# autowarefoundation/autoware_vision_pilot

Hardware: AMD Instinct MI355X
Metric: frames/sec (SceneSeg+Scene3D 1280x720, one camera per GPU: preprocess + shared encoder + 2 decoder(s) + decode per frame); p50 per-frame latency beside it (higher is better)
Workload: dtype fp16x3 (hi+lo fp16 pairs on the fp16 MFMA pipe, fp32 accumulate; fp32-class: floats within 1e-3 of the fp32 oracle, 0 class flips outside that float tolerance -- tie flips only, counted per pass in profiles/r06_parity_sweep.tsv)

## Files before the change

### autoware_vision_pilot_amd/csrc/engine_upconv.cpp

```cpp
#include "engine_internal.hpp"

namespace vp {

namespace {

inline void tap_of(int q, int tt, int* a, int* d) {
  const int hr = q + tt - 1;
  const int o = hr >= 0 ? hr / 2 : -1;
  *d = hr - 2 * o;
  *a = o + 1 - q;
}

inline void split_half_d(double v, double pre, half_t* hi, half_t* lo) {
  const double x = v * pre;
  if (!(std::fabs(x) <= 65504.0)) throw RangeError("composed up-sampling weight " + std::to_string(v) + " is outside the fp16 range the matrix pipe carries: re-scale the checkpoint");
  const half_t h = (half_t)x;
  *hi = h;
  *lo = truncate_lo((half_t)(x - (double)h));
}

}

void Engine::compose_upconv(const float* wt, const float* bt, const float* ws, const float* bs, const float* w3, const float* b3, int cin, int cm, int cout,
                            int cs, UpconvComposed* out) {
// ... 141 lines not shown
      }
      for (int t = 0; t < 9 && cs > 0; ++t) {
        const double* row = cw.ws.data() + ((size_t)t * cout + co) * cs;
        for (int c = 0; c < cs; ++c) amax = std::max(amax, std::fabs(row[c]));
      }
      const int sexp = prescale_exp((float)amax);
      const double pre = std::ldexp(1.0, sexp);
      post[(size_t)phase * coutw + co] = std::ldexp(1.0f, -sexp);
      for (int c = 0; c < n_chunks; ++c) {
        const UpconvChunk d = upconv_chunk(c, py, px, cin_v, cs_v);
        const int creal = d.skip ? cs : cin;
        for (int k = 0; k < d.nt; ++k) {
          const int a = d.a0 + (d.nb == 2 ? (k >> 1) : k), b = d.b0 + (d.nb == 2 ? (k & 1) : 0);
          const double* row;
          if (d.skip) {
            const int ty = d.qy != py ? 2 * a : 1, tx = d.qx != px ? 2 * b : 1;
            row = cw.ws.data() + ((size_t)(ty * 3 + tx) * cout + co) * cs;
          } else {
            row = cw.wx.data() + ((size_t)(phase * 4 + a * 2 + b) * cout + co) * cin;
          }
          for (int i = 0; i < chunk_w && chm * d.ch0 + i < creal; ++i) {
            const size_t dst = upconv_pack_index(phase, d.step0 + k, co, i & 31, S, coutw);
            if (x1) {
              half_t h, l;
              split_half_d(row[chm * d.ch0 + i], pre, &h, &l);
              (i >> 5 ? lo : hi)[dst] = h;
            } else {
              split_half_d(row[d.ch0 + i], pre, &hi[dst], &lo[dst]);
            }
          }
        }
      }
    }
  });
  Act* out = new_act(out_name.empty() ? name : out_name, cout, in->H * 2, in->W * 2);
  UpconvParams p{};
  p.in_hi = in->hi;
  p.in_lo = x1 ? nullptr : in->lo;
  p.sk_hi = skip_in ? skip_in->hi : nullptr;
  p.sk_lo = (skip_in && !x1) ? skip_in->lo : nullptr;
  p.H = in->H;
  p.W = in->W;
  p.Cin = cin_pad;
  p.Cs = cs_pad;
  p.w_hi = dupload(hi);
  p.w_lo = dupload(lo);
  wbytes_[1] += 2 * (hi.size() + lo.size());
  p.bias = dupload(bias);
  p.wscale = dupload(post);
  p.CoutW = coutw;
  p.Ncols = ncols;
  p.Cstore = out->C;
  p.out_hi = out->hi;
  p.out_lo = x1 ? nullptr : out->lo;
  p.act = (x1 && act == ACT_GELU) ? ACT_GELU_F16 : act;
  const long long t16 = (long long)((in->H + 15) / 16) * ((in->W + 15) / 16), t8 = (long long)((in->H + 7) / 8) * ((in->W + 15) / 16);
  const int n_co = coutw / 128;
  int sh = shape;
  {
    int ot = -1, on = 0;
    if (sh < 0 && plan_override(name, &ot, &on)) {
      sh = ot;
      if (on > 0 && nsplit <= 0) nsplit = on;
    }
  }
  if (sh < 0) {
    const double eff6 = (double)in->H * in->W / (double)(t16 * 256), eff7 = (double)in->H * in->W / (double)(t8 * 128);
    const char* e = dev_option("VP_UPCONV_SHAPE");
    sh = e ? std::atoi(e) : ((eff7 > 1.1 * eff6 || cin_pad <= 128) ? 7 : 6);
  }
  if (sh != 6 && sh != 7) throw std::invalid_argument("composed up-sampling stage: shape 6 (16x16 patches, 8 waves) or 7 (8x16 patches, 4 waves): " + name);
  const long long blocks = (sh == 6 ? t16 : t8) * 4 * n_co;
  int ns = nsplit;
  if (ns <= 0) {
    const long long slots = sh == 6 ? 256 : 512;
    ns = (int)std::max<long long>(1, slots / blocks);
    const double slice_mb = 4.0 * in->H * in->W * coutw * 4.0 / 1e6;
    while (ns > 1 && ns * slice_mb > 26.0) --ns;
    while (ns > 1 && S / ns < 12) --ns;
    if (const char* e = dev_option("VP_UPCONV_NSPLIT")) ns = std::max(1, std::atoi(e));
  }
  ns = std::max(1, std::min(ns, n_chunks));
  p.nsplit = ns;
  p.partial = ns > 1 ? static_cast<float*>(dalloc((size_t)ns * 4 * in->H * in->W * coutw * sizeof(float), false)) : nullptr;
  if (!upconv_supported(p, sh)) throw std::invalid_argument("composed up-sampling stage: shape not covered: " + name);
  Op op;
  op.name = name;
  op.kernel = std::string(x1 ? "upconv_x1" : "upconv_x3") + (sh == 6 ? "w8<co128,px256" : "w4<co128,px128") + (x1 ? ",k64>" : ">") + (ns > 1 ? "+splitk" : "");
  if (ns > 1) op.launch = "nsplit=" + std::to_string(ns);
  const double M2 = 4.0 * in->H * in->W;
  op.flops = 2.0 * (M2 * cin * cm + M2 * cs * cm + M2 * 9.0 * cm * cout);
  op.flops_executed = 2.0 * M2 * cout * (4.0 * cin + 9.0 * cs);
  op.bytes = (x1 ? 2.0 : 4.0) * ((M2 / 4 * cin + M2 * cs + M2 * cout) + cout * (16.0 * cin + 9.0 * cs));
  op.run = [p, sh](hipStream_t st) { return launch_upconv(p, sh, st); };
  ops_.push_back(std::move(op));
  return out;
}

}
```

### autoware_vision_pilot_amd/csrc/kernels.hpp

```cpp
#pragma once
#include "common.hpp"

namespace vp {

const char* dev_option(const char* key);
bool dev_option_is(const char* key, char first);

struct PreprocessParams {
  const uint8_t* frame;
  int stride;
  const int* xtab;
  const int* ytab;
  int out_h, out_w;
  int src_c[3];
  float mean[3], stdv[3];
  float* out;
  int norm_form;
};

struct PilResampleParams {
  const uint8_t* frame;
  int stride;
  int in_h, in_w, out_h, out_w;
  const int* hb;
// ... 126 lines not shown
  int N, K, act;
  unsigned act_rows;
  int rows_kernel;
  const float* partial;
  int nslab, Kstride;
  float inv_hw;
};

bool fc_rows_ok(const FcParams& p);

struct CtxConv1Params {
  const float* map;
  int H, W;
  const float* w;
  const float* b;
  ActView out;
  int act;
};

struct CtxExpConv1Params {
  FcParams fc;
  CtxConv1Params cv;
  int tile;
  int glanes;
};
bool ctx_exp_conv1_ok(const CtxExpConv1Params& p);
hipError_t launch_ctx_exp_conv1(const CtxExpConv1Params& p, hipStream_t st);

struct FusionParams {
  ActView f[5];
  int creal[5];
  int shift[5];
  ActView out;
  int Creal_out;
  int octets;
};
bool fusion_octets_ok(const FusionParams& p);

hipError_t launch_conv_gemm(const ConvGemmParams& p, int tile, int bk, bool split, hipStream_t st);
int conv_tile_co(int tile);
int conv_tile_px(int tile);
hipError_t launch_conv3x3_halo(const ConvGemmParams& p, int tile, bool split, hipStream_t st);
bool conv3x3_x3_supported(const ConvGemmParams& p, int shape);
hipError_t launch_conv3x3_x3(const ConvGemmParams& p, int shape, hipStream_t st);
int halo_tile_co(int tile);
int halo_tile_px(int tile);
int halo_tile_th(int tile);

int conv3x3_map_geometry(int H, int W);
bool conv3x3_map_shape_ok(int H, int W, int cin_pad, int coutw);
size_t conv3x3_map_pack_index(int co, int ci, int t, int cin_pad);
size_t conv3x3_map_pack_index_k32(int co, int ci, int t, int cin_pad);
bool conv3x3_map_supported(const ConvGemmParams& p);
hipError_t launch_conv3x3_map(const ConvGemmParams& p, hipStream_t st);
bool conv3x3_map2_shape_ok(int H, int W, int cin_pad, int coutw);
bool conv3x3_map2_supported(const ConvGemmParams& p);
size_t conv3x3_map2_pack_index(int co, int ci, int t, int cin_pad);
hipError_t launch_conv3x3_map2(const ConvGemmParams& p, hipStream_t st);
bool head_conv_supported(const ConvGemmParams& p);
hipError_t launch_head_conv(const ConvGemmParams& p, const void* zeros, hipStream_t st);
bool gemm_dma_shape_ok(int M, int ncols, int cin_pad, int cin2_pad, int cstore);
size_t gemm_dma_pack_index(int n, int k, int kw);
bool gemm_dma_supported(const ConvGemmParams& p, bool split);
hipError_t launch_gemm_dma(const ConvGemmParams& p, hipStream_t st);
bool convt_rs_supported(const ConvGemmParams& p, bool split);
int convt_rs_shape_case(int H, int W, int cin_pad, int cin2_pad, int ncols, int cstore);
hipError_t launch_convt_rs(const ConvGemmParams& p, hipStream_t st);
struct UpconvParams {
  const half_t* in_hi;
  const half_t* in_lo;
  const half_t* sk_hi;
  const half_t* sk_lo;
  int H, W, Cin, Cs;
  const half_t* w_hi;
  const half_t* w_lo;
  const float* bias;
  const float* wscale;
  int CoutW, Ncols, Cstore;
  half_t* out_hi;
  half_t* out_lo;
  int act;
  int nsplit;
  float* partial;
};
bool upconv_supported(const UpconvParams& p, int shape);
struct UpconvChunk {
  int skip, ch0, qy, qx, nt, nb, a0, b0, step0;
};
__host__ __device__ inline UpconvChunk upconv_chunk(int c, int py, int px, int cin_pad, int cs_pad) {
  const int kcx = cin_pad >> 5, kcs = cs_pad >> 5;
  UpconvChunk d;
  if (c < kcx || kcs == 0) {
    d.skip = 0; d.ch0 = c << 5; d.qy = 0; d.qx = 0; d.nt = 4; d.nb = 2; d.a0 = 0; d.b0 = 0; d.step0 = 4 * c;
    return d;
  }
  const int r = c - kcx, cls = r / kcs, cc = r - cls * kcs;
  d.skip = 1;
  d.ch0 = cc << 5;
  d.qy = cls < 2 ? 1 - py : py;
  d.qx = (cls & 1) ? px : 1 - px;
  const int na = d.qy != py ? 2 : 1;
  d.nb = d.qx != px ? 2 : 1;
  d.a0 = na == 2 ? 0 : 1 - py;
  d.b0 = d.nb == 2 ? 0 : 1 - px;
  d.nt = na * d.nb;
  const int cls_step0 = cls == 0 ? 0 : (cls == 1 ? 4 : (cls == 2 ? 6 : 8));
  d.step0 = 4 * kcx + cls_step0 * kcs + cc * d.nt;
  return d;
}
__host__ __device__ inline int upconv_chunks(int cin_pad, int cs_pad) { return (cin_pad >> 5) + 4 * (cs_pad >> 5); }
__host__ __device__ inline int upconv_steps(int cin_pad, int cs_pad) { return 4 * (cin_pad >> 5) + 9 * (cs_pad >> 5); }
inline size_t upconv_pack_index(int phase, int step, int co, int i, int steps, int coutw) {
  const int i_sw = ((((i & 31) >> 3) ^ ((co >> 2) & 3)) << 3) | (i & 7);
  return (((size_t)phase * steps + step) * coutw + co) * 32 + i_sw;
}
hipError_t launch_upconv(const UpconvParams& p, int shape, hipStream_t st);
struct ComposeGemmParams {
  const float* a[4];
  const float* b[4];
  int pairs, M, N, K;
  double* c;
};
hipError_t launch_compose_gemm(const ComposeGemmParams* groups_dev, int n_groups, int M, int N, hipStream_t st);
hipError_t launch_preprocess(const PreprocessParams& p, hipStream_t st);
hipError_t launch_pil_resample(const PilResampleParams& p, hipStream_t st);
hipError_t launch_stem(const StemParams& p, hipStream_t st);
hipError_t launch_dwconv(const DwParams& p, hipStream_t st);
bool mbconv_front_supported(const MbFrontParams& p);
hipError_t launch_mbconv_front(const MbFrontParams& p, hipStream_t st);
hipError_t launch_letterbox(const LetterboxParams& p, hipStream_t st);
hipError_t launch_detect_decode_nms(const DetectParams& p, hipStream_t st);
bool mbconv_back_supported(const MbBackParams& p);
hipError_t launch_mbconv_back(const MbBackParams& p, hipStream_t st);
hipError_t launch_pool_partial(const PoolParams& p, hipStream_t st);
hipError_t launch_zero_u64(unsigned long long* p, size_t n, hipStream_t st);
constexpr int kSeMaxReplicas = 64;
hipError_t launch_se_gate_scale(const SeParams& se, const ScaleWParams& sw, hipStream_t st);
hipError_t launch_fc(const FcParams& p, hipStream_t st);
hipError_t launch_ctx_conv1(const CtxConv1Params& p, hipStream_t st);
hipError_t launch_fusion(const FusionParams& p, hipStream_t st);
hipError_t launch_decode_mask(const float* logits, int C, int HW, int mode, uint8_t* out, hipStream_t st);
hipError_t launch_resize_nearest(const uint8_t* src, int sw, const int* ytab, const int* xtab, int oh, int ow, uint8_t* dst,
                                 hipStream_t st);
hipError_t launch_resize_bilinear_f32(const float* src, int sw, const int* yi, const float* yf, const int* xi, const float* xf,
                                      int oh, int ow, float* dst, hipStream_t st);
hipError_t launch_minmax_f32(const float* src, size_t n, unsigned* mm, hipStream_t st);
constexpr int VP_PROBE_BLOCKS = 64;
hipError_t launch_finite_probe(const float* src, size_t n, unsigned* flags, hipStream_t st);
hipError_t launch_depth_colorize(const float* src, size_t n, const unsigned* mm, const uint8_t* lut, uint8_t* dst, hipStream_t st);
hipError_t launch_viz_blend(const uint8_t* mask, int mw, const int* ytab, const int* xtab, const uint8_t* frame, int stride, int oh, int ow,
                            const uint8_t* lut, int frame_is_rgb, uint8_t* dst, hipStream_t st);
hipError_t launch_nchw_to_act(const float* src, int Creal, const ActView& a, hipStream_t st);
hipError_t launch_act_to_nchw(const ActView& a, int Creal, float* dst, hipStream_t st);

hipError_t launch_chan_copy(const ActView& src, int src_off, const ActView& dst, int dst_off, int nch, hipStream_t st);
hipError_t launch_maxpool5(const ActView& src, int src_off, const ActView& dst, int dst_off, int nch, hipStream_t st);
bool sppf_pool_ok(const ActView& src, const ActView& dst, int nch);
hipError_t launch_sppf_pool(const ActView& src, const ActView& dst, int nch, hipStream_t st);
struct AttnParams {
  ActView qkv;
  ActView out;
  ActView vout;
  int heads, dk, dv;
  float scale;
  int qblock;
};
bool attention_block_ok(const AttnParams& p);
hipError_t launch_attention(const AttnParams& p, hipStream_t st);
// ... 10 lines not shown
```

### autoware_vision_pilot_amd/csrc/kernels_upconv.hip

```cpp
#include <algorithm>
#include <cstdlib>

#include "conv_epilogue.hpp"
#include "lds_dma.hpp"

namespace vp {

namespace {

struct PixPhase {
  int y0, x0, H, W, py, px;
  __device__ __forceinline__ int operator()(int q) const {
    int rowbit, c;
    lane_to_px16(q & 31, rowbit, c);
    const int y = y0 + 2 * (q >> 5) + rowbit, x = x0 + c;
    return (y < H && x < W) ? (2 * y + py) * (2 * W) + 2 * x + px : -1;
  }
};
__device__ __forceinline__ int bias_class(int m, int H2, int W2) {
  const int Y = m / W2, X = m - Y * W2;
  return (Y == 0 ? 0 : (Y == H2 - 1 ? 2 : 1)) * 3 + (X == 0 ? 0 : (X == W2 - 1 ? 2 : 1));
}

}

#define VP_WAIT_VMCNT_RT(N)                       \
  do {                                            \
    const int n_ = (N);                           \
    if (n_ >= 16) { VP_WAIT_VMCNT(16); }          \
    else if (n_ >= 14) { VP_WAIT_VMCNT(14); }     \
    else if (n_ >= 12) { VP_WAIT_VMCNT(12); }     \
    else if (n_ >= 10) { VP_WAIT_VMCNT(10); }     \
    else if (n_ >= 8) { VP_WAIT_VMCNT(8); }       \
    else if (n_ >= 6) { VP_WAIT_VMCNT(6); }       \
    else if (n_ >= 4) { VP_WAIT_VMCNT(4); }       \
    else if (n_ >= 2) { VP_WAIT_VMCNT(2); }       \
    else { VP_WAIT_VMCNT(0); }                    \
  } while (0)

template <int CO_TILE, int TH, int WCO, int WPX, bool HDB, int ACT, bool SPLITK, bool X1 = false, int ABL = 0>
__global__ __launch_bounds__(64 * WCO * WPX, 2) void upconv_x3_kernel(const UpconvParams p) {
  constexpr int NTH = 64 * WCO * WPX;
  constexpr int TW = 16, ROWB = 80, HWD = TW + 2, HPX = (TH + 2) * HWD, PX = TH * TW;
  constexpr int HALO_BYTES = HPX * ROWB, WROW = 64, W_BYTES = CO_TILE * WROW;
  constexpr int HCHUNKS = HPX * 4, HP = (HCHUNKS + NTH - 1) / NTH;
  constexpr int MT = CO_TILE / WCO / 32, NT = PX / WPX / 32;
  constexpr int NHB = HDB ? 2 : 1;
  constexpr int PL = 2;
  constexpr int HSTRIDE = HALO_BYTES;
  static_assert(MT >= 1 && NT >= 1 && HP <= 3, "tile shape");
  extern __shared__ __attribute__((aligned(16))) char smem[];
  char* const halo_base = smem;
  char* const w_base = smem + NHB * PL * HSTRIDE;

  const int tid = threadIdx.x, lane = tid & 63, wave = tid >> 6;
  const int wco = wave / WPX, wpx = wave % WPX;
  const int tiles_x = (p.W + TW - 1) / TW;
  const int n_px_tiles = tiles_x * ((p.H + TH - 1) / TH);
  const int n_co_tiles = p.CoutW / CO_TILE;
  int vid;
  {
    const int nwg = gridDim.x, q = nwg >> 3, r = nwg & 7, xcd = blockIdx.x & 7;
    vid = (xcd < r ? xcd * (q + 1) : r * (q + 1) + (xcd - r) * q) + (blockIdx.x >> 3);
  }
  int tile_px, tile_co, phase, zsplit = 0;
  if constexpr (SPLITK) {
    tile_px = vid % n_px_tiles;
    int rest = vid / n_px_tiles;
    tile_co = rest % n_co_tiles;
    rest /= n_co_tiles;
    phase = rest & 3;
    zsplit = rest >> 2;
  } else {
    tile_co = vid % n_co_tiles;
    const int rest = vid / n_co_tiles;
    phase = rest & 3;
    tile_px = rest >> 2;
  }
  const int py = phase >> 1, px = phase & 1;
  const int tyi = tile_px / tiles_x, txi = tile_px - tyi * tiles_x;
  const int y0 = tyi * TH, x0 = txi * TW;
  const int co0 = tile_co * CO_TILE;
  const int CinV = X1 ? p.Cin >> 1 : p.Cin, CsV = X1 ? ((p.Cs + 63) >> 6) << 5 : p.Cs;
  constexpr int CHM = X1 ? 2 : 1;
  const half_t* const in_p1 = X1 ? p.in_hi + 32 : p.in_lo;
  const half_t* const sk_p1 = X1 ? p.sk_hi + 32 : p.sk_lo;
#define VP_SK_DEAD1(D) (X1 && (D).skip && CHM * (D).ch0 + 32 >= p.Cs)
  const int n_chunks = upconv_chunks(CinV, CsV);
  int cA = 0, cB = n_chunks;
  if constexpr (SPLITK) {
    cA = (int)(((long long)n_chunks * zsplit) / p.nsplit);
    cB = (int)(((long long)n_chunks * (zsplit + 1)) / p.nsplit);
  }

  const int h_lds0 = (tid >> 2) * ROWB + (tid & 3) * 16;
  constexpr int NW = NTH / 64, WPIECES = W_BYTES / 1024 / NW;
  static_assert(W_BYTES % (1024 * NW) == 0, "weight tile splits into 1 KiB pieces per wave");
  const size_t w_step = (size_t)p.CoutW * 32;
  typedef unsigned int u32x4 __attribute__((ext_vector_type(4)));
  const u32x4 zero4 = {0u, 0u, 0u, 0u};
  int b_ofs0;
  {
    int rowbit, c;
    lane_to_px16(lane & 31, rowbit, c);
    b_ofs0 = ((2 * (wpx * NT) + rowbit) * HWD + c) * ROWB + (lane >> 5) * 16;
  }
  const int a_swz = ((lane & 31) >> 2) & 3;
  const int a_ofs0 = (wco * 32 + (lane & 31)) * WROW + (((lane >> 5) ^ a_swz) << 4);

  int h_gx[HP], h_gs[HP];
#pragma unroll
  for (int pc = 0; pc < HP; ++pc) {
    const int hidx = tid + NTH * pc;
    const int hp = hidx >> 2, ch = hidx & 3;
    const int hy = hp / HWD, hx = hp - hy * HWD;
    const int gy = y0 - 1 + hy, gx = x0 - 1 + hx;
    const bool ok = hidx < HCHUNKS && (unsigned)gy < (unsigned)p.H && (unsigned)gx < (unsigned)p.W && hy >= py && hy <= py + TH && hx >= px && hx <= px + TW;
    h_gx[pc] = ok ? (gy * p.W + gx) * p.Cin + ch * 8 : -1;
    h_gs[pc] = ok ? (4 * gy * p.W + 2 * gx) * p.Cs + ch * 8 : -1;
  }
  const UpconvChunk dA = upconv_chunk(cA, py, px, CinV, CsV);
  const int S = (cB < n_chunks ? upconv_chunk(cB, py, px, CinV, CsV).step0 : upconv_steps(CinV, CsV)) - dA.step0;
  const size_t w_goff0 = ((size_t)phase * upconv_steps(CinV, CsV) + dA.step0) * w_step + co0 * 32 + wave * 512 + lane * 8;

  f32x16_t acc[MT][NT];
#pragma unroll
  for (int i = 0; i < MT; ++i)
#pragma unroll
    for (int j = 0; j < NT; ++j)
#pragma unroll
      for (int r = 0; r < 16; ++r) acc[i][j][r] = 0.0f;

  h8_t fa[2][MT], fal[2][MT], fb[2][NT], fbl[2][NT];
  u32x4 rh_hi[HP], rh_lo[HP];
#pragma unroll
  for (int r = 0; r < HP; ++r) rh_hi[r] = rh_lo[r] = zero4;

#define VP_DMA_W(WOFS, SIDX)                                                                 \
  if (!(ABL & 128) || (SIDX) < 2) {                                                          \
    const size_t base_ = (size_t)(SIDX) * w_step + w_goff0;                                  \
    char* dst_ = w_base + (WOFS) + wave * 1024;                                              \
    _Pragma("unroll") for (int pc = 0; pc < WPIECES; ++pc) {                                 \
      VP_GLOBAL_LOAD_LDS16(p.w_hi + base_ + pc * NW * 512, dst_ + pc * NW * 1024);           \
      VP_GLOBAL_LOAD_LDS16(p.w_lo + base_ + pc * NW * 512, dst_ + W_BYTES + pc * NW * 1024); \
    }                                                                                        \
  }
#define VP_LOAD_H(D)                                                                         \
  if (!(ABL & 1) || abl_prologue) {                                                          \
    const half_t* sh_ = (D).skip ? p.sk_hi : p.in_hi;                                        \
    const half_t* sl_ = (D).skip ? (VP_SK_DEAD1(D) ? p.sk_hi : sk_p1) : in_p1;               \
    const int add_ = (D).skip ? ((D).qy * 2 * p.W + (D).qx) * p.Cs + CHM * (D).ch0 : CHM * (D).ch0; \
    _Pragma("unroll") for (int pc = 0; pc < HP; ++pc) {                                      \
      const int g_ = (D).skip ? h_gs[pc] : h_gx[pc];                                         \
      const int o_ = (g_ >= 0 ? g_ + add_ : 0);                                              \
      rh_hi[pc] = *reinterpret_cast<const u32x4*>(sh_ + o_);                                 \
      rh_lo[pc] = *reinterpret_cast<const u32x4*>(sl_ + o_);                                 \
    }                                                                                        \
  }
#define VP_STORE_H(BUF, DEAD1)                                                               \
  if (!(ABL & 1) || abl_prologue)                                                            \
  _Pragma("unroll") for (int pc = 0; pc < HP; ++pc) {                                        \
    if (tid + NTH * pc < HCHUNKS) {                                                          \
      char* dst_ = halo_base + (BUF) * PL * HSTRIDE + h_lds0 + pc * (NTH / 4) * ROWB;        \
      *reinterpret_cast<u32x4*>(dst_) = h_gx[pc] >= 0 ? rh_hi[pc] : zero4;                   \
      *reinterpret_cast<u32x4*>(dst_ + HSTRIDE) = (h_gx[pc] >= 0 && !(DEAD1)) ? rh_lo[pc] : zero4; \
    }                                                                                        \
  }
#define VP_READ_FRAGS(SET, WPTR, HPTR, TAPOFS)                                               \
  {                                                                                          \
    const char* wsrc_ = (WPTR) + (a_ofs0 ^ ((SET) * 32));                                    \
    _Pragma("unroll") for (int i = 0; i < MT; ++i) {                                         \
      fa[SET][i] = *reinterpret_cast<const h8_t*>(wsrc_ + i * WCO * 32 * WROW);              \
      fal[SET][i] = *reinterpret_cast<const h8_t*>(wsrc_ + W_BYTES + i * WCO * 32 * WROW);   \
    }                                                                                        \
    const char* hsrc_ = (HPTR) + b_ofs0 + (TAPOFS) + (SET) * 32;                             \
    _Pragma("unroll") for (int j = 0; j < NT; ++j) {                                         \
      fb[SET][j] = *reinterpret_cast<const h8_t*>(hsrc_ + j * 2 * HWD * ROWB);               \
      fbl[SET][j] = *reinterpret_cast<const h8_t*>(hsrc_ + HSTRIDE + j * 2 * HWD * ROWB);    \
    }                                                                                        \
  }
#define VP_MFMA_RANGE(SET, Q0, Q1)                                                           \
  _Pragma("unroll") for (int q_ = (Q0); q_ < (Q1); ++q_) {                                   \
    const int i = q_ / NT, j = q_ % NT;                                                      \
    if constexpr ((ABL & 2) != 0) { acc[i][j][0] += (float)fa[SET][i][0] + (float)fal[SET][i][1] + (float)fb[SET][j][2] + (float)fbl[SET][j][3]; continue; } \
    if constexpr (X1) {                      \
      acc[i][j] = __builtin_amdgcn_mfma_f32_32x32x16_f16(fa[SET][i], fb[SET][j], acc[i][j], 0, 0, 0);   \
      acc[i][j] = __builtin_amdgcn_mfma_f32_32x32x16_f16(fal[SET][i], fbl[SET][j], acc[i][j], 0, 0, 0); \
      continue;                                                                              \
    }                                                                                        \
    acc[i][j] = __builtin_amdgcn_mfma_f32_32x32x16_f16(fal[SET][i], fb[SET][j], acc[i][j], 0, 0, 0); \
    acc[i][j] = __builtin_amdgcn_mfma_f32_32x32x16_f16(fa[SET][i], fbl[SET][j], acc[i][j], 0, 0, 0); \
    acc[i][j] = __builtin_amdgcn_mfma_f32_32x32x16_f16(fa[SET][i], fb[SET][j], acc[i][j], 0, 0, 0);  \
  }
#define VP_TAP_OFS(D, K) ((((py + (D).a0 + ((D).nb == 2 ? ((K) >> 1) : (K))) * HWD) + px + (D).b0 + ((D).nb == 2 ? ((K) & 1) : 0)) * ROWB)

  bool abl_prologue = true;
  VP_LOAD_H(dA)
  VP_STORE_H(0, VP_SK_DEAD1(dA))
  VP_DMA_W(0, 0)
  if (S > 1) VP_DMA_W(PL * W_BYTES, 1)
  VP_WAIT_VMCNT(0);
  __syncthreads();
  UpconvChunk d = dA;
  UpconvChunk dn = dA;
  if (cA + 1 < cB) {
    dn = upconv_chunk(cA + 1, py, px, CinV, CsV);
    VP_LOAD_H(dn)
  }
  VP_READ_FRAGS(0, w_base, halo_base, VP_TAP_OFS(d, 0))
  abl_prologue = false;

  int c = cA, t = 0, s = 0, hb = 0;
  int w_cur = 0, w_nxt = PL * W_BYTES, w_fre = 2 * PL * W_BYTES;
#define VP_STEP(KIND, PREVLD)                                                                \
  {                                                                                          \
    const int tap_cur_ = VP_TAP_OFS(d, t);                                                   \
    const int tap_nxt_ = (KIND) == 0 ? VP_TAP_OFS(d, t + 1) : ((KIND) == 3 ? tap_cur_ : VP_TAP_OFS(dn, 0)); \
    const char* hbuf = halo_base + (HDB ? hb : 0) * PL * HSTRIDE;                            \
    const char* hbuf_next = (HDB && (KIND) != 0) ? halo_base + (hb ^ 1) * PL * HSTRIDE : hbuf; \
     \
     \
     \
    if constexpr (HDB && ((KIND) == 1 || (KIND) == 2)) { VP_STORE_H(hb ^ 1, VP_SK_DEAD1(dn)) }   \
     \
    if (s + 2 < S) VP_DMA_W(w_fre, s + 2)                                                    \
    __builtin_amdgcn_sched_barrier(0);                                                       \
    VP_MFMA_RANGE(0, 0, MT * NT / 2)                                                         \
    __builtin_amdgcn_sched_barrier(0);                                                       \
    VP_READ_FRAGS(1, w_base + w_cur, hbuf, tap_cur_)                                         \
    __builtin_amdgcn_sched_barrier(0);   \
    UpconvChunk dnn = dn;                                                                    \
    if constexpr (HDB && (KIND) == 1) {                                                      \
      dnn = upconv_chunk(c + 2, py, px, CinV, CsV);                                        \
      VP_LOAD_H(dnn)                                                                         \
    }                                                                                        \
    VP_MFMA_RANGE(0, MT * NT / 2, MT * NT)                                                   \
    __builtin_amdgcn_sched_barrier(0);                                                       \
     \
     \
    {                                                                                        \
      const int dma_n = s + 2 < S ? PL * WPIECES : 0;                                        \
      const int ld_prev = ((PREVLD) && t == 0) ? PL * HP : 0;                                \
      const int ld_this = (HDB && (KIND) == 1) ? PL * HP : 0;                                \
      VP_WAIT_VMCNT_RT(dma_n + ld_prev + ld_this);                                           \
    }                                                                                        \
     \
    VP_LDS_BARRIER();                                                                        \
    if constexpr (!HDB && ((KIND) == 1 || (KIND) == 2)) {                                    \
       \
       \
      VP_STORE_H(0, VP_SK_DEAD1(dn))                                                         \
      VP_LDS_BARRIER();                                                                      \
      if constexpr ((KIND) == 1) {                                                           \
        dnn = upconv_chunk(c + 2, py, px, CinV, CsV);                                      \
        VP_LOAD_H(dnn)                                                                       \
      }                                                                                      \
    }                                                                                        \
           \
    VP_READ_FRAGS(0, w_base + w_nxt, hbuf_next, tap_nxt_)                                    \
    __builtin_amdgcn_sched_barrier(0);                                                       \
    VP_MFMA_RANGE(1, 0, MT * NT)                                                             \
    __builtin_amdgcn_sched_barrier(0);                                                       \
                                    \
    {                                                                                        \
      const int w_old = w_cur;                                                               \
      w_cur = w_nxt;                                                                         \
      w_nxt = w_fre;                                                                         \
      w_fre = w_old;                                                                         \
    }                                                                                        \
    ++s;                                                                                     \
    if constexpr ((KIND) == 0) {                                                             \
      ++t;                                                                                   \
    } else {                                                                                 \
      ++c;                                                                                   \
      t = 0;                                                                                 \
      d = dn;                                                                                \
      dn = dnn;                                                                              \
      hb ^= 1;                                                                               \
    }                                                                                        \
  }
  while (c + 2 < cB) {
    while (t + 1 < d.nt) VP_STEP(0, true)
    VP_STEP(1, true)
  }
  if (c + 1 < cB) {
    while (t + 1 < d.nt) VP_STEP(0, true)
    VP_STEP(2, true)
  }
  while (t + 1 < d.nt) VP_STEP(0, false)
  VP_STEP(3, false)
#undef VP_STEP
#undef VP_SK_DEAD1
#undef VP_TAP_OFS
#undef VP_MFMA_RANGE
#undef VP_READ_FRAGS
#undef VP_STORE_H
#undef VP_LOAD_H
#undef VP_DMA_W

  const PixPhase pix{y0, x0, p.H, p.W, py, px};
  if constexpr ((ABL & 16) != 0) {
    if (p.H == -12345) {
#pragma unroll
      for (int i = 0; i < MT; ++i)
#pragma unroll
        for (int j = 0; j < NT; ++j)
#pragma unroll
          for (int r = 0; r < 16; ++r) p.partial[(i * NT + j) * 16 + r + tid * 64] = acc[i][j][r];
    }
    return;
  }
  if constexpr (SPLITK) {
    const int M2 = 4 * p.H * p.W;
#pragma unroll
    for (int j = 0; j < NT; ++j) {
      const int m = pix((wpx * NT + j) * 32 + (lane & 31));
      if (m < 0) continue;
      float* row = p.partial + ((size_t)zsplit * M2 + m) * p.CoutW + co0 + 4 * (lane >> 5);
#pragma unroll
      for (int i = 0; i < MT; ++i)
#pragma unroll
        for (int g = 0; g < 4; ++g) {
          const f32x4_t v = {acc[i][j][4 * g + 0], acc[i][j][4 * g + 1], acc[i][j][4 * g + 2], acc[i][j][4 * g + 3]};
          *reinterpret_cast<f32x4_t*>(row + (i * WCO + wco) * 32 + 8 * g) = v;
        }
    }
    return;
  } else {
    constexpr int PITCH = CO_TILE * 2 + 16, STAGE_PLANE = PX * PITCH;
    static_assert(PL * STAGE_PLANE <= NHB * PL * HSTRIDE + 3 * PL * W_BYTES, "stage fits the main buffers");
    const float* const wsc = p.wscale + (size_t)phase * p.CoutW + co0;
    f32x4_t bb[NT][MT][4], sc[MT][4];
    int qpix[NT];
#pragma unroll
    for (int j = 0; j < NT; ++j) {
      qpix[j] = (wpx * NT + j) * 32 + (lane & 31);
      const int m = pix(qpix[j]);
      const float* const bsrc = p.bias + (size_t)(m >= 0 ? bias_class(m, 2 * p.H, 2 * p.W) : 4) * p.CoutW + co0;
#pragma unroll
      for (int i = 0; i < MT; ++i)
#pragma unroll
        for (int g = 0; g < 4; ++g) bb[j][i][g] = *reinterpret_cast<const f32x4_t*>(bsrc + (i * WCO + wco) * 32 + 4 * (lane >> 5) + 8 * g);
    }
#pragma unroll
    for (int i = 0; i < MT; ++i)
#pragma unroll
      for (int g = 0; g < 4; ++g) sc[i][g] = *reinterpret_cast<const f32x4_t*>(wsc + (i * WCO + wco) * 32 + 4 * (lane >> 5) + 8 * g);
    __syncthreads();
#pragma unroll
    for (int j = 0; j < NT; ++j) {
#pragma unroll
      for (int i = 0; i < MT; ++i) {
        const int cl = (i * WCO + wco) * 32 + 4 * (lane >> 5);
        char* row = smem + qpix[j] * PITCH + cl * 2;
#pragma unroll
        for (int g = 0; g < 4; ++g) {
          h4_t h, l;
#pragma unroll
          for (int r = 0; r < 4; ++r) {
            const float x = apply_act(fmaf(acc[i][j][4 * g + r], sc[i][g][r], bb[j][i][g][r]), ACT);
            h[r] = (half_t)x;
            if constexpr (!X1) l[r] = (half_t)(x - (float)h[r]);
          }
          *reinterpret_cast<h4_t*>(row + g * 16) = h;
          if constexpr (!X1) *reinterpret_cast<h4_t*>(row + STAGE_PLANE + g * 16) = l;
        }
      }
    }
    __syncthreads();
    constexpr int CPR = CO_TILE / 8, RPI = NTH / CPR;
    static_assert(NTH % CPR == 0 && PX % RPI == 0, "row loop shape");
    const int c8 = tid % CPR, r0 = tid / CPR;
    const int co = co0 + c8 * 8;
    if (co >= p.Ncols) return;
#pragma unroll 4
    for (int r = r0; r < PX; r += RPI) {
      const int m = pix(r);
      if (m < 0) continue;
      if constexpr ((ABL & 32) != 0) { if (p.H != -12345) continue; }
      const size_t o = (size_t)m * p.Cstore + co;
      *reinterpret_cast<h8_t*>(p.out_hi + o) = *reinterpret_cast<const h8_t*>(smem + r * PITCH + c8 * 16);
      if constexpr (!X1) *reinterpret_cast<h8_t*>(p.out_lo + o) = *reinterpret_cast<const h8_t*>(smem + STAGE_PLANE + r * PITCH + c8 * 16);
    }
  }
}

__global__ __launch_bounds__(256) void upconv_finish_kernel(const UpconvParams p) {
  const int H2 = 2 * p.H, W2 = 2 * p.W, M2 = H2 * W2;
  const int groups = p.Ncols >> 3;
  const long long t = (long long)blockIdx.x * 256 + threadIdx.x;
  if (t >= (long long)M2 * groups) return;
  const int m = (int)(t / groups), co = (int)(t % groups) * 8;
  float v[8] = {0.f, 0.f, 0.f, 0.f, 0.f, 0.f, 0.f, 0.f};
  for (int z = 0; z < p.nsplit; ++z) {
    const float* src = p.partial + ((size_t)z * M2 + m) * p.CoutW + co;
    const f32x4_t q0 = *reinterpret_cast<const f32x4_t*>(src), q1 = *reinterpret_cast<const f32x4_t*>(src + 4);
#pragma unroll
    for (int r = 0; r < 4; ++r) {
      v[r] += q0[r];
      v[4 + r] += q1[r];
    }
  }
  const int Y = m / W2, X = m - Y * W2;
  const int phase = (Y & 1) * 2 + (X & 1);
  const float* b = p.bias + (size_t)bias_class(m, H2, W2) * p.CoutW + co;
  const float* s = p.wscale + (size_t)phase * p.CoutW + co;
  h8_t hi, lo;
#pragma unroll
  for (int r = 0; r < 8; ++r) {
    const float x = apply_act(fmaf(v[r], s[r], b[r]), p.act);
    hi[r] = (half_t)x;
    lo[r] = (half_t)(x - (float)hi[r]);
  }
  const size_t o = (size_t)m * p.Cstore + co;
  *reinterpret_cast<h8_t*>(p.out_hi + o) = hi;
  if (p.out_lo) *reinterpret_cast<h8_t*>(p.out_lo + o) = lo;
}

bool upconv_supported(const UpconvParams& p, int shape) {
  if (shape != 6 && shape != 7) return false;
  const bool x1 = p.in_lo == nullptr;
  if (!(p.in_hi && p.w_hi && p.w_lo && p.bias && p.wscale && p.out_hi && (x1 ? p.out_lo == nullptr : p.out_lo != nullptr))) return false;
  if (p.H < 1 || p.W < 1 || p.Cin < (x1 ? 64 : 32) || p.Cin % (x1 ? 64 : 32) != 0 || p.Cs % 32 != 0 || p.Cs < 0) return false;
  if (p.Cs > 0 && !(p.sk_hi && (x1 ? p.sk_lo == nullptr : p.sk_lo != nullptr))) return false;
  if (p.CoutW % 128 != 0 || p.Ncols % 8 != 0 || p.Ncols > p.CoutW || p.Cstore < p.Ncols) return false;
  if (!(p.act == (x1 ? ACT_GELU_F16 : ACT_GELU) || p.act == ACT_NONE)) return false;
  if (p.nsplit < 1 || p.nsplit > (x1 ? upconv_chunks(p.Cin >> 1, ((p.Cs + 63) >> 6) << 5) : upconv_chunks(p.Cin, p.Cs))) return false;
  if (p.nsplit > 1 && !p.partial) return false;
  if ((long long)p.H * p.W * p.Cin >= (1ll << 31) || 4ll * p.H * p.W * std::max(p.Cs, 1) >= (1ll << 31) || 4ll * p.H * p.W * p.Cstore >= (1ll << 31)) return false;
  return true;
}

template <int TH, int WPX, bool HDB, bool X1>
static hipError_t launch_upconv_cfg(const UpconvParams& p, hipStream_t st) {
  constexpr int CO = 128;
  constexpr int lds = (HDB ? 2 : 1) * 2 * ((TH + 2) * 18 * 80) + 6 * (CO * 64);
  static_assert(lds <= 160 * 1024, "LDS budget");
  constexpr int GELU = X1 ? ACT_GELU_F16 : ACT_GELU;
  const bool gelu = p.act == GELU, sk = p.nsplit > 1;
  auto k = sk ? upconv_x3_kernel<CO, TH, 2, WPX, HDB, ACT_NONE, true, X1>
              : (gelu ? upconv_x3_kernel<CO, TH, 2, WPX, HDB, GELU, false, X1> : upconv_x3_kernel<CO, TH, 2, WPX, HDB, ACT_NONE, false, X1>);
  static LdsAttrOnce attr_once[3];
  if (hipError_t e = set_max_dynamic_lds(attr_once[sk ? 2 : gelu], reinterpret_cast<const void*>(k), lds); e != hipSuccess) return e;
  dim3 grid(((p.H + TH - 1) / TH) * ((p.W + 15) / 16) * 4 * (p.CoutW / CO) * p.nsplit);
  hipLaunchKernelGGL(k, grid, dim3(64 * 2 * WPX), lds, st, p);
  hipError_t e = hipGetLastError();
  if (e != hipSuccess || !sk) return e;
  const long long n = 4ll * p.H * p.W * (p.Ncols >> 3);
  hipLaunchKernelGGL(upconv_finish_kernel, dim3((unsigned)((n + 255) / 256)), dim3(256), 0, st, p);
  return hipGetLastError();
}

hipError_t launch_upconv(const UpconvParams& p, int shape, hipStream_t st) {
  if (!upconv_supported(p, shape)) return hipErrorInvalidValue;
  if (p.in_lo == nullptr) {
    if (shape == 6) return launch_upconv_cfg<16, 4, true, true>(p, st);
    return launch_upconv_cfg<8, 2, false, true>(p, st);
  }
  if (shape == 6) return launch_upconv_cfg<16, 4, true, false>(p, st);
  return launch_upconv_cfg<8, 2, false, false>(p, st);
}

__global__ __launch_bounds__(256) void compose_gemm_kernel(const ComposeGemmParams* groups, int tiles_n) {
  __shared__ float As[16][64 + 4], Bs[16][64 + 4];
  const ComposeGemmParams& g = groups[blockIdx.y];
  const int tm = blockIdx.x / tiles_n, tn = blockIdx.x - tm * tiles_n;
  const int tid = threadIdx.x, tx = tid & 15, ty = tid >> 4;
  const int lrow = tid >> 2, lk = (tid & 3) * 4;
  double acc[4][4];
#pragma unroll
  for (int i = 0; i < 4; ++i)
#pragma unroll
    for (int j = 0; j < 4; ++j) acc[i][j] = 0.0;
  for (int pr = 0; pr < g.pairs; ++pr) {
    const float* A = g.a[pr];
    const float* B = g.b[pr];
    for (int k0 = 0; k0 < g.K; k0 += 16) {
#pragma unroll
      for (int e = 0; e < 4; ++e) {
        const int k = k0 + lk + e;
        const int ma = tm * 64 + lrow, nb = tn * 64 + lrow;
        As[lk + e][lrow] = (ma < g.M && k < g.K) ? A[(size_t)ma * g.K + k] : 0.0f;
        Bs[lk + e][lrow] = (nb < g.N && k < g.K) ? B[(size_t)nb * g.K + k] : 0.0f;
      }
      __syncthreads();
#pragma unroll
      for (int k = 0; k < 16; ++k) {
        double a[4], b[4];
#pragma unroll
        for (int i = 0; i < 4; ++i) {
          a[i] = (double)As[k][ty * 4 + i];
          b[i] = (double)Bs[k][tx * 4 + i];
        }
#pragma unroll
        for (int i = 0; i < 4; ++i)
#pragma unroll
          for (int j = 0; j < 4; ++j) acc[i][j] = fma(a[i], b[j], acc[i][j]);
      }
      __syncthreads();
    }
  }
#pragma unroll
  for (int i = 0; i < 4; ++i)
#pragma unroll
    for (int j = 0; j < 4; ++j) {
      const int m = tm * 64 + ty * 4 + i, n = tn * 64 + tx * 4 + j;
      if (m < g.M && n < g.N) g.c[(size_t)m * g.N + n] = acc[i][j];
    }
}

hipError_t launch_compose_gemm(const ComposeGemmParams* groups_dev, int n_groups, int M, int N, hipStream_t st) {
  const int tiles_m = (M + 63) / 64, tiles_n = (N + 63) / 64;
  hipLaunchKernelGGL(compose_gemm_kernel, dim3(tiles_m * tiles_n, n_groups), dim3(256), 0, st, groups_dev, tiles_n);
  return hipGetLastError();
}

}
```

### autoware_vision_pilot_amd/csrc/options.cpp

```cpp
#include <atomic>
#include <cstring>
#include <deque>
#include <map>
#include <mutex>
#include <string>

#include "../../include/vp_hip.h"
#include "kernels.hpp"

namespace vp {
namespace {
std::mutex g_mu;
std::atomic<int> g_count{0};
std::map<std::string, const char*> g_opts;
std::deque<std::string> g_arena;
bool g_version_stale = true;
std::deque<std::string> g_versions;

const char* const kKeys[] = {"VP_MBCONV_FUSE", "VP_MBCONV_BACK", "VP_PROJ_SPLIT", "VP_FUSE_DECODE", "VP_AUTOTUNE", "VP_HEAD_CONV", "VP_CONVT_RS",
                             "VP_CONV3X3", "VP_HEAD_TILE5", "VP_X3_TILE", "VP_X3_MIN_WGS", "VP_MAP3X3", "VP_NSPLIT_PCT", "VP_NSPLIT_FORCE", "VP_X3_C64",
                             "VP_GEMM_DMA", "VP_GEMM_DMA_NSPLIT", "VP_CONVT_TILE", "VP_CONVT_BK", "VP_FUSE_SKIP", "VP_CONVT_RS_GROUPS", "VP_F16_BIG",
                             "VP_CTX3", "VP_MAP_TAPSPLIT", "VP_ATTN_BLOCK", "VP_F16_MAP", "VP_MAP_NSPLIT_PCT", "VP_MAP2", "VP_MAP2_SLOTS", "VP_X3_T16", "VP_MAP2_CAP_MB", "VP_MAP2_MIN_REGIONS", "VP_CTX_FUSE", "VP_MAP_MAX_M", "VP_F16_MIN_WGS", "VP_CONVT_RS_GROUPS_K288", "VP_PLAN_TARGET", "VP_UPCONV", "VP_UPCONV_SHAPE", "VP_UPCONV_NSPLIT", "VP_PLAN_OVERRIDE", "VP_WLO_KEEP_BITS", "VP_UPCONV_F16"};
}

const char* dev_option(const char* key) {
  if (g_count.load(std::memory_order_acquire) == 0) return nullptr;
  std::lock_guard<std::mutex> lk(g_mu);
  auto it = g_opts.find(key);
  return it == g_opts.end() ? nullptr : it->second;
}
bool dev_option_is(const char* key, char first) {
  const char* v = dev_option(key);
  return v != nullptr && v[0] == first;
}

}

extern "C" {

int vp_set_option(const char* key, const char* value) {
  if (!key) return VP_ERR_ARG;
  bool known = false;
  for (const char* k : vp::kKeys) known = known || std::strcmp(k, key) == 0;
  if (!known) return VP_ERR_ARG;
  if (value && std::strcmp(key, "VP_PLAN_TARGET") == 0 && std::strcmp(value, "latency") != 0 && std::strcmp(value, "throughput") != 0) return VP_ERR_ARG;
  std::lock_guard<std::mutex> lk(vp::g_mu);
  if (!value) {
    vp::g_opts.erase(key);
  } else {
    vp::g_arena.emplace_back(value);
    vp::g_opts[key] = vp::g_arena.back().c_str();
  }
  vp::g_version_stale = true;
  vp::g_count.store((int)vp::g_opts.size(), std::memory_order_release);
  return VP_OK;
}

const char* vp_get_option(const char* key) { return key ? vp::dev_option(key) : nullptr; }

void vp_clear_options(void) {
  std::lock_guard<std::mutex> lk(vp::g_mu);
  vp::g_opts.clear();
  vp::g_version_stale = true;
  vp::g_count.store(0, std::memory_order_release);
}

const char* vp_version(void) {
  std::lock_guard<std::mutex> lk(vp::g_mu);
  if (vp::g_version_stale) {
    std::string s = "libvp_hip 0.5 (gfx950; options:";
    if (vp::g_opts.empty()) s += " none";
    for (const auto& kv : vp::g_opts) s += std::string(" ") + kv.first + "=" + kv.second;
    s += ")";
    if (vp::g_versions.empty() || vp::g_versions.back() != s) vp::g_versions.push_back(s);
    vp::g_version_stale = false;
  }
  return vp::g_versions.back().c_str();
}

}
```

Measured before the change: 546.8.

## Add compact row-major pixel-run tiling to composed up-sampling kernel

Adds a compact mode to the x3 up-sampling kernel in which each workgroup takes a contiguous run of row-major pixels instead of a 2D 16-wide tile. The aim is to avoid the padded, partly empty tiles that occur when the width is not a multiple of 16, and to cut the workgroup count. The halo becomes a row-strip layout with per-lane B offsets, and waves with no valid pixels skip their fragment loads and MFMAs. Compact mode turns on by default only when the run count is below the 2D tile count and the halo fits in the capacity check. The cost is more index arithmetic, an irregular halo gather, and a larger halo for the 8-row shape.

```diff
diff --git a/autoware_vision_pilot_amd/csrc/engine_upconv.cpp b/autoware_vision_pilot_amd/csrc/engine_upconv.cpp
--- a/autoware_vision_pilot_amd/csrc/engine_upconv.cpp
+++ b/autoware_vision_pilot_amd/csrc/engine_upconv.cpp
@@ -247,6 +247,12 @@
   }
   ns = std::max(1, std::min(ns, n_chunks));
   p.nsplit = ns;
+  {
+    const long long px = sh == 6 ? 256 : 128, runs = ((long long)in->H * in->W + px - 1) / px;
+    const char* e = dev_option("VP_UPCONV_COMPACT");
+    const bool want = e ? e[0] == '1' : runs < (sh == 6 ? t16 : t8);
+    p.compact = (!x1 && want && upconv_compact_fits(in->H, in->W, sh)) ? 1 : 0;
+  }
   p.partial = ns > 1 ? static_cast<float*>(dalloc((size_t)ns * 4 * in->H * in->W * coutw * sizeof(float), false)) : nullptr;
   if (!upconv_supported(p, sh)) throw std::invalid_argument("composed up-sampling stage: shape not covered: " + name);
   Op op;
diff --git a/autoware_vision_pilot_amd/csrc/kernels.hpp b/autoware_vision_pilot_amd/csrc/kernels.hpp
--- a/autoware_vision_pilot_amd/csrc/kernels.hpp
+++ b/autoware_vision_pilot_amd/csrc/kernels.hpp
@@ -232,8 +232,10 @@
   int act;
   int nsplit;
   float* partial;
+  int compact;
 };
 bool upconv_supported(const UpconvParams& p, int shape);
+bool upconv_compact_fits(int H, int W, int shape);
 struct UpconvChunk {
   int skip, ch0, qy, qx, nt, nb, a0, b0, step0;
 };
diff --git a/autoware_vision_pilot_amd/csrc/kernels_upconv.hip b/autoware_vision_pilot_amd/csrc/kernels_upconv.hip
--- a/autoware_vision_pilot_amd/csrc/kernels_upconv.hip
+++ b/autoware_vision_pilot_amd/csrc/kernels_upconv.hip
@@ -17,6 +17,19 @@
     return (y < H && x < W) ? (2 * y + py) * (2 * W) + 2 * x + px : -1;
   }
 };
+struct PixRun {
+  int kA, kE, W, py, px;
+  __device__ __forceinline__ int operator()(int q) const {
+    int rowbit, c;
+    lane_to_px16(q & 31, rowbit, c);
+    const int k = kA + (q >> 5) * 32 + 16 * rowbit + c;
+    if (k >= kE) return -1;
+    const int y = k / W, x = k - y * W;
+    return (2 * y + py) * (2 * W) + 2 * x + px;
+  }
+};
+constexpr int upconv_halo_bytes(int TH, bool CPT) { return (CPT && TH == 8) ? 192 * 80 : (TH + 2) * 18 * 80; }
+constexpr int upconv_halo_capacity(int nth) { return 3 * nth / 4; }
 __device__ __forceinline__ int bias_class(int m, int H2, int W2) {
   const int Y = m / W2, X = m - Y * W2;
   return (Y == 0 ? 0 : (Y == H2 - 1 ? 2 : 1)) * 3 + (X == 0 ? 0 : (X == W2 - 1 ? 2 : 1));
@@ -38,11 +51,11 @@
     else { VP_WAIT_VMCNT(0); }                    \
   } while (0)
 
-template <int CO_TILE, int TH, int WCO, int WPX, bool HDB, int ACT, bool SPLITK, bool X1 = false, int ABL = 0>
+template <int CO_TILE, int TH, int WCO, int WPX, bool HDB, int ACT, bool SPLITK, bool X1 = false, int ABL = 0, bool CPT = false>
 __global__ __launch_bounds__(64 * WCO * WPX, 2) void upconv_x3_kernel(const UpconvParams p) {
   constexpr int NTH = 64 * WCO * WPX;
   constexpr int TW = 16, ROWB = 80, HWD = TW + 2, HPX = (TH + 2) * HWD, PX = TH * TW;
-  constexpr int HALO_BYTES = HPX * ROWB, WROW = 64, W_BYTES = CO_TILE * WROW;
+  constexpr int HALO_BYTES = upconv_halo_bytes(TH, CPT), WROW = 64, W_BYTES = CO_TILE * WROW;
   constexpr int HCHUNKS = HPX * 4, HP = (HCHUNKS + NTH - 1) / NTH;
   constexpr int MT = CO_TILE / WCO / 32, NT = PX / WPX / 32;
   constexpr int NHB = HDB ? 2 : 1;
@@ -56,7 +69,7 @@
   const int tid = threadIdx.x, lane = tid & 63, wave = tid >> 6;
   const int wco = wave / WPX, wpx = wave % WPX;
   const int tiles_x = (p.W + TW - 1) / TW;
-  const int n_px_tiles = tiles_x * ((p.H + TH - 1) / TH);
+  const int n_px_tiles = CPT ? (p.H * p.W + PX - 1) / PX : tiles_x * ((p.H + TH - 1) / TH);
   const int n_co_tiles = p.CoutW / CO_TILE;
   int vid;
   {
@@ -80,6 +93,10 @@
   const int py = phase >> 1, px = phase & 1;
   const int tyi = tile_px / tiles_x, txi = tile_px - tyi * tiles_x;
   const int y0 = tyi * TH, x0 = txi * TW;
+  const int kA = tile_px * PX, kE = min(kA + PX, p.H * p.W);
+  const int yA = kA / p.W, xA = kA - yA * p.W, yE = (kE - 1) / p.W, xE = (kE - 1) - yE * p.W;
+  const int hrp = CPT ? p.W * ROWB + 256 : HWD * ROWB;
+  const int tpy = CPT ? 0 : py, tpx = CPT ? 0 : px;
   const int co0 = tile_co * CO_TILE;
   const int CinV = X1 ? p.Cin >> 1 : p.Cin, CsV = X1 ? ((p.Cs + 63) >> 6) << 5 : p.Cs;
   constexpr int CHM = X1 ? 2 : 1;
@@ -100,22 +117,46 @@
   typedef unsigned int u32x4 __attribute__((ext_vector_type(4)));
   const u32x4 zero4 = {0u, 0u, 0u, 0u};
   int b_ofs0;
+  int b_ofs[NT];
+  int nlj = NT;
   {
     int rowbit, c;
     lane_to_px16(lane & 31, rowbit, c);
     b_ofs0 = ((2 * (wpx * NT) + rowbit) * HWD + c) * ROWB + (lane >> 5) * 16;
+    if constexpr (CPT) {
+#pragma unroll
+      for (int j = 0; j < NT; ++j) {
+        int k = kA + (wpx * NT + j) * 32 + 16 * rowbit + c;
+        if (k >= kE) k = kA;
+        const int y = k / p.W, x = k - y * p.W;
+        b_ofs[j] = (y - yA) * hrp + (x - xA) * ROWB + (lane >> 5) * 16;
+      }
+      nlj = __builtin_amdgcn_readfirstlane(min(NT, max(0, (kE - kA + 31) / 32 - wpx * NT)));
+    }
   }
   const int a_swz = ((lane & 31) >> 2) & 3;
   const int a_ofs0 = (wco * 32 + (lane & 31)) * WROW + (((lane >> 5) ^ a_swz) << 4);
 
-  int h_gx[HP], h_gs[HP];
+  int h_gx[HP], h_gs[HP], h_ls[HP];
 #pragma unroll
   for (int pc = 0; pc < HP; ++pc) {
     const int hidx = tid + NTH * pc;
     const int hp = hidx >> 2, ch = hidx & 3;
-    const int hy = hp / HWD, hx = hp - hy * HWD;
-    const int gy = y0 - 1 + hy, gx = x0 - 1 + hx;
-    const bool ok = hidx < HCHUNKS && (unsigned)gy < (unsigned)p.H && (unsigned)gx < (unsigned)p.W && hy >= py && hy <= py + TH && hx >= px && hx <= px + TW;
+    int gy, gx;
+    bool ok;
+    if constexpr (CPT) {
+      const int gw = p.W + 2, lg = py * gw + xA + px + hp, cnt = (yE - yA + 1) * gw + xE - xA + 2;
+      const int r = lg / gw, cc = lg - r * gw;
+      gy = yA - 1 + r;
+      gx = cc - 1;
+      ok = hp < cnt && (unsigned)gy < (unsigned)p.H && (unsigned)gx < (unsigned)p.W;
+      h_ls[pc] = hp < cnt ? (r - py) * hrp + (cc - xA - px) * ROWB + ch * 16 : -1;
+    } else {
+      const int hy = hp / HWD, hx = hp - hy * HWD;
+      gy = y0 - 1 + hy;
+      gx = x0 - 1 + hx;
+      ok = hidx < HCHUNKS && (unsigned)gy < (unsigned)p.H && (unsigned)gx < (unsigned)p.W && hy >= py && hy <= py + TH && hx >= px && hx <= px + TW;
+    }
     h_gx[pc] = ok ? (gy * p.W + gx) * p.Cin + ch * 8 : -1;
     h_gs[pc] = ok ? (4 * gy * p.W + 2 * gx) * p.Cs + ch * 8 : -1;
   }
@@ -160,8 +201,8 @@
 #define VP_STORE_H(BUF, DEAD1)                                                               \
   if (!(ABL & 1) || abl_prologue)                                                            \
   _Pragma("unroll") for (int pc = 0; pc < HP; ++pc) {                                        \
-    if (tid + NTH * pc < HCHUNKS) {                                                          \
-      char* dst_ = halo_base + (BUF) * PL * HSTRIDE + h_lds0 + pc * (NTH / 4) * ROWB;        \
+    if (CPT ? h_ls[pc] >= 0 : tid + NTH * pc < HCHUNKS) {                                    \
+      char* dst_ = halo_base + (BUF) * PL * HSTRIDE + (CPT ? h_ls[pc] : h_lds0 + pc * (NTH / 4) * ROWB); \
       *reinterpret_cast<u32x4*>(dst_) = h_gx[pc] >= 0 ? rh_hi[pc] : zero4;                   \
       *reinterpret_cast<u32x4*>(dst_ + HSTRIDE) = (h_gx[pc] >= 0 && !(DEAD1)) ? rh_lo[pc] : zero4; \
     }                                                                                        \
@@ -169,19 +210,30 @@
 #define VP_READ_FRAGS(SET, WPTR, HPTR, TAPOFS)                                               \
   {                                                                                          \
     const char* wsrc_ = (WPTR) + (a_ofs0 ^ ((SET) * 32));                                    \
+    if (!CPT || nlj > 0)                                                                     \
     _Pragma("unroll") for (int i = 0; i < MT; ++i) {                                         \
       fa[SET][i] = *reinterpret_cast<const h8_t*>(wsrc_ + i * WCO * 32 * WROW);              \
       fal[SET][i] = *reinterpret_cast<const h8_t*>(wsrc_ + W_BYTES + i * WCO * 32 * WROW);   \
     }                                                                                        \
-    const char* hsrc_ = (HPTR) + b_ofs0 + (TAPOFS) + (SET) * 32;                             \
-    _Pragma("unroll") for (int j = 0; j < NT; ++j) {                                         \
-      fb[SET][j] = *reinterpret_cast<const h8_t*>(hsrc_ + j * 2 * HWD * ROWB);               \
-      fbl[SET][j] = *reinterpret_cast<const h8_t*>(hsrc_ + HSTRIDE + j * 2 * HWD * ROWB);    \
+    if constexpr (CPT) {                                                                     \
+      const char* hsrc_ = (HPTR) + (TAPOFS) + (SET) * 32;                                    \
+      _Pragma("unroll") for (int j = 0; j < NT; ++j) {                                       \
+        if (j >= nlj) continue;                                                              \
+        fb[SET][j] = *reinterpret_cast<const h8_t*>(hsrc_ + b_ofs[j]);                       \
+        fbl[SET][j] = *reinterpret_cast<const h8_t*>(hsrc_ + HSTRIDE + b_ofs[j]);            \
+      }                                                                                      \
+    } else {                                                                                 \
+      const char* hsrc_ = (HPTR) + b_ofs0 + (TAPOFS) + (SET) * 32;                           \
+      _Pragma("unroll") for (int j = 0; j < NT; ++j) {                                       \
+        fb[SET][j] = *reinterpret_cast<const h8_t*>(hsrc_ + j * 2 * HWD * ROWB);             \
+        fbl[SET][j] = *reinterpret_cast<const h8_t*>(hsrc_ + HSTRIDE + j * 2 * HWD * ROWB);  \
+      }                                                                                      \
     }                                                                                        \
   }
 #define VP_MFMA_RANGE(SET, Q0, Q1)                                                           \
   _Pragma("unroll") for (int q_ = (Q0); q_ < (Q1); ++q_) {                                   \
     const int i = q_ / NT, j = q_ % NT;                                                      \
+    if constexpr (CPT) { if (j >= nlj) continue; }        \
     if constexpr ((ABL & 2) != 0) { acc[i][j][0] += (float)fa[SET][i][0] + (float)fal[SET][i][1] + (float)fb[SET][j][2] + (float)fbl[SET][j][3]; continue; } \
     if constexpr (X1) {                      \
       acc[i][j] = __builtin_amdgcn_mfma_f32_32x32x16_f16(fa[SET][i], fb[SET][j], acc[i][j], 0, 0, 0);   \
@@ -192,7 +244,7 @@
     acc[i][j] = __builtin_amdgcn_mfma_f32_32x32x16_f16(fa[SET][i], fbl[SET][j], acc[i][j], 0, 0, 0); \
     acc[i][j] = __builtin_amdgcn_mfma_f32_32x32x16_f16(fa[SET][i], fb[SET][j], acc[i][j], 0, 0, 0);  \
   }
-#define VP_TAP_OFS(D, K) ((((py + (D).a0 + ((D).nb == 2 ? ((K) >> 1) : (K))) * HWD) + px + (D).b0 + ((D).nb == 2 ? ((K) & 1) : 0)) * ROWB)
+#define VP_TAP_OFS(D, K) ((tpy + (D).a0 + ((D).nb == 2 ? ((K) >> 1) : (K))) * hrp + (tpx + (D).b0 + ((D).nb == 2 ? ((K) & 1) : 0)) * ROWB)
 
   bool abl_prologue = true;
   VP_LOAD_H(dA)
@@ -298,7 +350,10 @@
 #undef VP_LOAD_H
 #undef VP_DMA_W
 
-  const PixPhase pix{y0, x0, p.H, p.W, py, px};
+  const auto pix = [&] {
+    if constexpr (CPT) return PixRun{kA, kE, p.W, py, px};
+    else return PixPhase{y0, x0, p.H, p.W, py, px};
+  }();
   if constexpr ((ABL & 16) != 0) {
     if (p.H == -12345) {
 #pragma unroll
@@ -417,8 +472,21 @@
   if (p.out_lo) *reinterpret_cast<h8_t*>(p.out_lo + o) = lo;
 }
 
+bool upconv_compact_fits(int H, int W, int shape) {
+  if ((shape != 6 && shape != 7) || H < 1 || W < 1 || (long long)H * W >= (1 << 24)) return false;
+  const int PX = shape == 6 ? 256 : 128, nth = shape == 6 ? 512 : 256, th = shape == 6 ? 16 : 8;
+  for (int kA = 0; kA < H * W; kA += PX) {
+    const int kE = std::min(kA + PX, H * W), yA = kA / W, xA = kA - yA * W, yE = (kE - 1) / W, xE = (kE - 1) - yE * W;
+    const long long cnt = (long long)(yE - yA + 1) * (W + 2) + xE - xA + 2;
+    const long long bytes = (long long)(yE - yA + 1) * (W * 80 + 256) + (xE - xA + 1) * 80 + 80;
+    if (cnt > upconv_halo_capacity(nth) || bytes > upconv_halo_bytes(th, true)) return false;
+  }
+  return true;
+}
+
 bool upconv_supported(const UpconvParams& p, int shape) {
   if (shape != 6 && shape != 7) return false;
+  if (p.compact && (p.in_lo == nullptr || !upconv_compact_fits(p.H, p.W, shape))) return false;
   const bool x1 = p.in_lo == nullptr;
   if (!(p.in_hi && p.w_hi && p.w_lo && p.bias && p.wscale && p.out_hi && (x1 ? p.out_lo == nullptr : p.out_lo != nullptr))) return false;
   if (p.H < 1 || p.W < 1 || p.Cin < (x1 ? 64 : 32) || p.Cin % (x1 ? 64 : 32) != 0 || p.Cs % 32 != 0 || p.Cs < 0) return false;
@@ -431,18 +499,19 @@
   return true;
 }
 
-template <int TH, int WPX, bool HDB, bool X1>
+template <int TH, int WPX, bool HDB, bool X1, bool CPT = false>
 static hipError_t launch_upconv_cfg(const UpconvParams& p, hipStream_t st) {
   constexpr int CO = 128;
-  constexpr int lds = (HDB ? 2 : 1) * 2 * ((TH + 2) * 18 * 80) + 6 * (CO * 64);
-  static_assert(lds <= 160 * 1024, "LDS budget");
+  constexpr int lds = (HDB ? 2 : 1) * 2 * upconv_halo_bytes(TH, CPT) + 6 * (CO * 64);
+  static_assert(lds <= (TH == 8 ? 80 : 160) * 1024, "LDS budget (the 4-wave shape: two workgroups per CU)");
   constexpr int GELU = X1 ? ACT_GELU_F16 : ACT_GELU;
   const bool gelu = p.act == GELU, sk = p.nsplit > 1;
-  auto k = sk ? upconv_x3_kernel<CO, TH, 2, WPX, HDB, ACT_NONE, true, X1>
-              : (gelu ? upconv_x3_kernel<CO, TH, 2, WPX, HDB, GELU, false, X1> : upconv_x3_kernel<CO, TH, 2, WPX, HDB, ACT_NONE, false, X1>);
+  auto k = sk ? upconv_x3_kernel<CO, TH, 2, WPX, HDB, ACT_NONE, true, X1, 0, CPT>
+              : (gelu ? upconv_x3_kernel<CO, TH, 2, WPX, HDB, GELU, false, X1, 0, CPT> : upconv_x3_kernel<CO, TH, 2, WPX, HDB, ACT_NONE, false, X1, 0, CPT>);
   static LdsAttrOnce attr_once[3];
   if (hipError_t e = set_max_dynamic_lds(attr_once[sk ? 2 : gelu], reinterpret_cast<const void*>(k), lds); e != hipSuccess) return e;
-  dim3 grid(((p.H + TH - 1) / TH) * ((p.W + 15) / 16) * 4 * (p.CoutW / CO) * p.nsplit);
+  const int n_px = CPT ? (p.H * p.W + TH * 16 - 1) / (TH * 16) : ((p.H + TH - 1) / TH) * ((p.W + 15) / 16);
+  dim3 grid(n_px * 4 * (p.CoutW / CO) * p.nsplit);
   hipLaunchKernelGGL(k, grid, dim3(64 * 2 * WPX), lds, st, p);
   hipError_t e = hipGetLastError();
   if (e != hipSuccess || !sk) return e;
@@ -456,6 +525,10 @@
   if (p.in_lo == nullptr) {
     if (shape == 6) return launch_upconv_cfg<16, 4, true, true>(p, st);
     return launch_upconv_cfg<8, 2, false, true>(p, st);
+  }
+  if (p.compact) {
+    if (shape == 6) return launch_upconv_cfg<16, 4, true, false, true>(p, st);
+    return launch_upconv_cfg<8, 2, false, false, true>(p, st);
   }
   if (shape == 6) return launch_upconv_cfg<16, 4, true, false>(p, st);
   return launch_upconv_cfg<8, 2, false, false>(p, st);
diff --git a/autoware_vision_pilot_amd/csrc/options.cpp b/autoware_vision_pilot_amd/csrc/options.cpp
--- a/autoware_vision_pilot_amd/csrc/options.cpp
+++ b/autoware_vision_pilot_amd/csrc/options.cpp
@@ -20,7 +20,7 @@
 const char* const kKeys[] = {"VP_MBCONV_FUSE", "VP_MBCONV_BACK", "VP_PROJ_SPLIT", "VP_FUSE_DECODE", "VP_AUTOTUNE", "VP_HEAD_CONV", "VP_CONVT_RS",
                              "VP_CONV3X3", "VP_HEAD_TILE5", "VP_X3_TILE", "VP_X3_MIN_WGS", "VP_MAP3X3", "VP_NSPLIT_PCT", "VP_NSPLIT_FORCE", "VP_X3_C64",
                              "VP_GEMM_DMA", "VP_GEMM_DMA_NSPLIT", "VP_CONVT_TILE", "VP_CONVT_BK", "VP_FUSE_SKIP", "VP_CONVT_RS_GROUPS", "VP_F16_BIG",
-                             "VP_CTX3", "VP_MAP_TAPSPLIT", "VP_ATTN_BLOCK", "VP_F16_MAP", "VP_MAP_NSPLIT_PCT", "VP_MAP2", "VP_MAP2_SLOTS", "VP_X3_T16", "VP_MAP2_CAP_MB", "VP_MAP2_MIN_REGIONS", "VP_CTX_FUSE", "VP_MAP_MAX_M", "VP_F16_MIN_WGS", "VP_CONVT_RS_GROUPS_K288", "VP_PLAN_TARGET", "VP_UPCONV", "VP_UPCONV_SHAPE", "VP_UPCONV_NSPLIT", "VP_PLAN_OVERRIDE", "VP_WLO_KEEP_BITS", "VP_UPCONV_F16"};
+                             "VP_CTX3", "VP_MAP_TAPSPLIT", "VP_ATTN_BLOCK", "VP_F16_MAP", "VP_MAP_NSPLIT_PCT", "VP_MAP2", "VP_MAP2_SLOTS", "VP_X3_T16", "VP_MAP2_CAP_MB", "VP_MAP2_MIN_REGIONS", "VP_CTX_FUSE", "VP_MAP_MAX_M", "VP_F16_MIN_WGS", "VP_CONVT_RS_GROUPS_K288", "VP_PLAN_TARGET", "VP_UPCONV", "VP_UPCONV_SHAPE", "VP_UPCONV_NSPLIT", "VP_PLAN_OVERRIDE", "VP_WLO_KEEP_BITS", "VP_UPCONV_F16", "VP_UPCONV_COMPACT"};
 }
 
 const char* dev_option(const char* key) {
```

After: 563.1, median of 6. 1.03x the previous value.
